# esologic/GANce

Hardware: AMD Instinct MI355X
Metric: synthesized frames/sec at 1024x1024 config-f (higher is better)
Workload: dtype f32 (bf16x3 split operands, 6 terms, fp32 accumulate)

## Files before the change

gance_amd/csrc/upfir_split.hip:

```cpp

#include <hip/hip_runtime.h>

#include <algorithm>
#include <cstdlib>
#include <cstring>
#include <type_traits>

#include "kernels.h"

#ifndef GANCE_UPFIRS_ABLATE
#define GANCE_UPFIRS_ABLATE 0
#endif

namespace gance {

namespace {

typedef float f32x4 __attribute__((ext_vector_type(4)));
typedef float f32x2 __attribute__((ext_vector_type(2)));
typedef unsigned u32x4 __attribute__((ext_vector_type(4)));
typedef unsigned u32x2 __attribute__((ext_vector_type(2)));
typedef __bf16 bf16x8 __attribute__((ext_vector_type(8)));
typedef __bf16 bf16x2 __attribute__((ext_vector_type(2)));
typedef __attribute__((address_space(3))) void* lds_ptr_t;

constexpr int kBM = 16;
constexpr int kKC = 32;
constexpr int kSW = 64;
constexpr int kTH = 8;
constexpr int kRows = kTH + 1;
constexpr int kPlanes = 12;
constexpr int kPlaneStride = 80;
constexpr int kSlotUnits = kPlanes * kPlaneStride;
constexpr int kRing = 3;
constexpr int kHaloCols = 4;
constexpr int kHaloUnits = kRows * kHaloCols * kPlanes;
constexpr int kHaloTasks = kRows * kHaloCols * 4;
#ifndef GANCE_UPFIRS_WEAVE
#define GANCE_UPFIRS_WEAVE 2
#endif
#ifndef GANCE_UPFIRS_MIN_SEG_ROWS
#define GANCE_UPFIRS_MIN_SEG_ROWS 16
#endif
#ifndef GANCE_UPFIRS_DEPTH
#define GANCE_UPFIRS_DEPTH 6
#endif
constexpr int kDepth = GANCE_UPFIRS_DEPTH;
constexpr int kCarryRows = 3;
constexpr int kPassCh = 4;
constexpr int kPassRows = 8;
constexpr float kSqrt2f = 1.4142135623730951f;
static_assert((2 * kRows) % kDepth == 0 && kDepth + 2 < kRows && kRows % kRing == 0, "ring slots and staging registers rotate with the unrolled rows of a chunk pair");

template <int NT>
struct Geo {
    static constexpr int kSW = 64 / NT;
    static constexpr int kBMB = kBM * NT;
    static constexpr int kTC = kSW / 16;
    static constexpr int kPW = 4 / NT;
    static constexpr int kTW = 2 * kSW + 4;
    static constexpr int kCG = kSW / 2;
    static constexpr int kRG = 64 / NT / kCG;
    static constexpr int kFR = kPassRows / kRG;
    static constexpr int kWin = kFR + 3;
    static constexpr int kCarryFloats = kBMB * kCarryRows * kTW;
    static constexpr int kStageFloats = kPassCh * NT * kPassRows * kTW;
    static constexpr int kNzPieces = 2 * kPassRows * 2 * kSW / 256;
    static constexpr int kWUnits = NT == 1 ? 27 * 64 : 0;
};

constexpr size_t kRingBytes = (size_t)kRing * kSlotUnits * 16;
constexpr size_t kHaloBytes = (size_t)2 * kHaloUnits * 16;
template <int NT>
constexpr size_t lds_bytes(int cin) {
    using G = Geo<NT>;
    return kRingBytes + kHaloBytes + (size_t)G::kWUnits * 16 +
           sizeof(float) * ((size_t)G::kStageFloats + G::kNzPieces * 256 + G::kCarryFloats + cin + 3 * G::kBMB);
}

__host__ __device__ constexpr int tap_cls(int t) { return t < 4 ? 0 : (t < 6 ? 1 : (t < 8 ? 2 : 3)); }
__host__ __device__ constexpr int tap_dy(int t) { return (t == 2 || t == 3 || t == 5) ? 1 : 0; }
__host__ __device__ constexpr int tap_dx(int t) { return (t == 1 || t == 3 || t == 7) ? 1 : 0; }

__device__ __forceinline__ void lds_barrier() {
    asm volatile("s_waitcnt lgkmcnt(0)" ::: "memory");
    __builtin_amdgcn_s_barrier();
    asm volatile("" ::: "memory");
}

__device__ __forceinline__ int fresh_lane() {
    int l;
    asm volatile("v_mbcnt_lo_u32_b32 %0, -1, 0\n\tv_mbcnt_hi_u32_b32 %0, -1, %0" : "=v"(l));
    return l;
}

__device__ __forceinline__ int ring_column(int P) {
    return ((P >> 2) & 3) | ((((P >> 4) ^ P) & 1) << 2) | (((P >> 1) & 1) << 3) | ((P & 1) << 4) | (P & 32);
}
constexpr int kEdgeColumn = 64;

__device__ __forceinline__ void split_pair(float a, float b, unsigned& p0, unsigned& p1, unsigned& p2) {
    auto pack = [](float lo, float hi) { return __builtin_bit_cast(unsigned, __builtin_convertvector(f32x2{lo, hi}, bf16x2)); };
    p0 = pack(a, b);
    const float ra = a - __builtin_bit_cast(float, p0 << 16), rb = b - __builtin_bit_cast(float, p0 & 0xffff0000u);
    p1 = pack(ra, rb);
    const float sa = ra - __builtin_bit_cast(float, p1 << 16), sb = rb - __builtin_bit_cast(float, p1 & 0xffff0000u);
    p2 = pack(sa, sb);
}

__device__ __forceinline__ void split_unit(const unsigned (&raw)[8], u32x4 (&part)[3]) {
    unsigned w[3][4];
    if (GANCE_UPFIRS_ABLATE & 1) {
#pragma unroll
        for (int q = 0; q < 3; ++q) part[q] = u32x4{raw[q], raw[q + 1], raw[q + 2], raw[q + 3]};
        return;
    }
#pragma unroll
    for (int e = 0; e < 4; ++e) split_pair(__builtin_bit_cast(float, raw[2 * e]), __builtin_bit_cast(float, raw[2 * e + 1]), w[0][e], w[1][e], w[2][e]);
#pragma unroll
    for (int q = 0; q < 3; ++q) part[q] = u32x4{w[q][0], w[q][1], w[q][2], w[q][3]};
}

}

template <int NT, bool kPre, bool kNoise>
__device__ __forceinline__ void upfirs_body(const UpFirArgs& p) {
    using G = Geo<NT>;
    constexpr int kSW = G::kSW, kBMB = G::kBMB, kTC = G::kTC, kPW = G::kPW, kTW = G::kTW, kCG = G::kCG, kRG = G::kRG, kFR = G::kFR,
                  kWin = G::kWin, kCarryFloats = G::kCarryFloats, kStageFloats = G::kStageFloats, kNzPieces = G::kNzPieces;
    extern __shared__ __attribute__((aligned(16))) unsigned char smem_raw[];
    u32x4* const ring = reinterpret_cast<u32x4*>(smem_raw);
    u32x4* const halo = ring + kRing * kSlotUnits;
    u32x4* const w_lds = halo + 2 * kHaloUnits;
    float* const stage = reinterpret_cast<float*>(w_lds + G::kWUnits);
    float* const nz_lds = stage + kStageFloats;
    float* const carry = nz_lds + kNzPieces * 256;
    float* const s_lds = carry + kCarryFloats;
    float* const d_lds = s_lds + (kPre ? 0 : p.Cin);
    float* const b_lds = d_lds + kBMB;
    float* const sn_lds = b_lds + kBMB;

    const int tid = threadIdx.x;
    const int wave = __builtin_amdgcn_readfirstlane(tid >> 6);
    const int lane = tid & 63;
    const int n16 = lane & 15, kg = lane >> 4;
    const int ct = NT == 1 ? 0 : wave / kTC, tc = NT == 1 ? wave : wave % kTC;

    int id;
    {
        const int v = blockIdx.x, nwg = p.total_blocks;
        const int q = nwg >> 3, r = nwg & 7, xcd = v & 7;
        id = (xcd < r ? xcd * (q + 1) : r * (q + 1) + (xcd - r) * q) + (v >> 3);
    }
    const int m_tile = id % p.m_tiles;
    id /= p.m_tiles;
    const int strip = id % p.strips;
    id /= p.strips;
    const int seg = id % p.segs;
    const int b = id / p.segs;
    const int m0 = m_tile * kBMB;
    const int X0 = strip * kSW;
    const int H = p.H, W = p.W;
    const int Hp = H + 2, Wp = W + 8;
    const int HpWp4 = Hp * Wp * 4;
    const int chunks = p.Cin / kKC;
    const int steps = H / kTH;
    const int s_begin = seg * (p.rows_per_seg / kTH), s_end = s_begin + p.rows_per_seg / kTH;
    const int s_first = seg > 0 ? s_begin - 1 : s_begin;

    const __amdgpu_buffer_rsrc_t x_rsrc =
        __builtin_amdgcn_make_buffer_rsrc((void*)(p.x + (size_t)b * p.x_b_stride), 0, p.Cin * Hp * Wp * 4, 0x00020000);
    const __amdgpu_buffer_rsrc_t w_rsrc = __builtin_amdgcn_make_buffer_rsrc(
        (void*)(reinterpret_cast<const unsigned char*>(p.w) + (size_t)(m_tile * NT + ct) * chunks * 27 * 1024), 0, chunks * 27 * 1024, 0x00020000);

    const int st_pair = lane >> 4, st_g = lane & 15;
    u32x4* const ring_w = ring + wave * kPlaneStride + ring_column(4 * st_g + st_pair);
    unsigned* const ring_wn = reinterpret_cast<unsigned*>(ring + wave * kPlaneStride + ring_column(NT == 2 ? 2 * st_g + (st_pair & 1) : st_g)) +
                              (NT == 2 ? 2 * (st_pair >> 1) : st_pair);
    const int m_pos = 16 * tc + n16;
    const u32x4* const ring_r0 = ring + kg * kPlaneStride + ring_column(m_pos);
    const u32x4* const ring_r1 = ring + kg * kPlaneStride + (m_pos > 0 ? ring_column(m_pos - 1) : kEdgeColumn);
    const bool edge_copy = wave == 3 && lane < kPlanes;
    const int e_unit = lane % kPlanes;
    u32x4* const ring_e = ring + (e_unit >> 2) * 4 * kPlaneStride + (e_unit & 3) * kPlaneStride + (edge_copy ? kEdgeColumn : 66 + wave);
    const u32x4* const halo_e = halo + e_unit;
    const u32x4* const halo_r = halo + ((n16 & 7) * kHaloCols + 2 * (n16 >> 3)) * kPlanes + kg;
    const u32x4* const halo_f = halo + ((kRows - 1) * kHaloCols + 2 * (n16 >> 3)) * kPlanes + kg;
    const int st_voff = (2 * st_pair * Hp * Wp + X0 + 4 + kPW * st_g) * 4;
    unsigned st[kDepth][8];
    auto stage_load = [&](unsigned(&dst)[8], int chunk, int brow, bool in_loop = false) {
        if ((GANCE_UPFIRS_ABLATE & 4) && in_loop) return;
        const int soff = ((chunk * kKC + wave * 8) * Hp + brow) * Wp * 4;
#pragma unroll
        for (int e = 0; e < 2; ++e) {
            if constexpr (kPW == 4) {
                const u32x4 q4 = __builtin_amdgcn_raw_buffer_load_b128(x_rsrc, st_voff, soff + e * HpWp4, 0);
#pragma unroll
                for (int c = 0; c < 4; ++c) dst[2 * c + e] = q4[c];
            } else if constexpr (kPW == 2) {
                const u32x2 q2 = __builtin_amdgcn_raw_buffer_load_b64(x_rsrc, st_voff, soff + e * HpWp4, 0);
                dst[e] = q2[0];
                dst[2 + e] = q2[1];
            } else {
                dst[e] = __builtin_amdgcn_raw_buffer_load_b32(x_rsrc, st_voff, soff + e * HpWp4, 0);
            }
        }
    };
    auto scale_pair = [&](unsigned(&raw)[8], int chunk) {
        if constexpr (!kPre) {
            const f32x2 s2 = *reinterpret_cast<const f32x2*>(s_lds + chunk * kKC + 8 * wave + 2 * st_pair);
#pragma unroll
            for (int c = 0; c < kPW; ++c) {
                raw[2 * c] = __builtin_bit_cast(unsigned, __builtin_bit_cast(float, raw[2 * c]) * s2[0]);
                raw[2 * c + 1] = __builtin_bit_cast(unsigned, __builtin_bit_cast(float, raw[2 * c + 1]) * s2[1]);
            }
        }
    };
    auto transpose_rows = [](u32x4& u) {
        auto a02 = __builtin_amdgcn_permlane32_swap(u[0], u[2], false, false);
        auto a13 = __builtin_amdgcn_permlane32_swap(u[1], u[3], false, false);
        auto b01 = __builtin_amdgcn_permlane16_swap(a02[0], a13[0], false, false);
        auto b23 = __builtin_amdgcn_permlane16_swap(a02[1], a13[1], false, false);
        u = u32x4{b01[0], b01[1], b23[0], b23[1]};
    };
    auto scale8 = [&](unsigned(&raw)[8], int chunk, int group) {
        if constexpr (!kPre) {
            const f32x4 s0 = *reinterpret_cast<const f32x4*>(s_lds + chunk * kKC + group * 8);
            const f32x4 s1 = *reinterpret_cast<const f32x4*>(s_lds + chunk * kKC + group * 8 + 4);
#pragma unroll
            for (int e = 0; e < 4; ++e) {
                raw[e] = __builtin_bit_cast(unsigned, __builtin_bit_cast(float, raw[e]) * s0[e]);
                raw[4 + e] = __builtin_bit_cast(unsigned, __builtin_bit_cast(float, raw[4 + e]) * s1[e]);
            }
        }
    };
    auto stage_store = [&](unsigned(&raw)[8], int slot, int chunk) {
        scale_pair(raw, chunk);
        if constexpr (NT == 1) {
            u32x4 part[3];
            split_unit(raw, part);
#pragma unroll
            for (int q = 0; q < 3; ++q) transpose_rows(part[q]);
#pragma unroll
            for (int q = 0; q < 3; ++q)
                if (!(GANCE_UPFIRS_ABLATE & 16)) ring_w[slot * kSlotUnits + q * 4 * kPlaneStride] = part[q];
        } else {
            unsigned w[3][kPW];
#pragma unroll
            for (int c = 0; c < kPW; ++c) split_pair(__builtin_bit_cast(float, raw[2 * c]), __builtin_bit_cast(float, raw[2 * c + 1]), w[0][c], w[1][c], w[2][c]);
#pragma unroll
            for (int q = 0; q < 3; ++q) {
                unsigned* const dst = ring_wn + 4 * (slot * kSlotUnits + q * 4 * kPlaneStride);
                if constexpr (NT == 2) {
                    const auto s = __builtin_amdgcn_permlane16_swap(w[q][0], w[q][1], false, false);
                    *reinterpret_cast<u32x2*>(dst) = u32x2{s[0], s[1]};
                } else {
                    *dst = w[q][0];
                }
            }
        }
    };
    auto edge_store = [&](int slot, int hbuf, int hrow) { if (!(GANCE_UPFIRS_ABLATE & 64)) ring_e[slot * kSlotUnits] = halo_e[hbuf * kHaloUnits + (hrow * kHaloCols + 1) * kPlanes]; };
    const int h_task = tid < kHaloTasks ? tid : tid - kHaloTasks;
    const int h_col = h_task & 3, h_kg = (h_task >> 2) & 3, h_row = h_task >> 4;
    const int h_voff = ((h_kg * 8 * Hp + h_row) * Wp + X0 + 2 + (h_col & 1) + (h_col >> 1) * (kSW + 1)) * 4;
    u32x4* const halo_w = halo + (h_row * kHaloCols + h_col) * kPlanes + h_kg;
    unsigned hraw[8];
    auto halo_load = [&](int step, int chunk) {
        const int soff = (chunk * kKC * Hp + kTH * step) * Wp * 4;
#pragma unroll
        for (int e = 0; e < 8; ++e) hraw[e] = __builtin_amdgcn_raw_buffer_load_b32(x_rsrc, h_voff, soff + e * HpWp4, 0);
    };
    auto halo_store = [&](int chunk, int buf) {
        scale8(hraw, chunk, h_kg);
        u32x4 part[3];
        split_unit(hraw, part);
#pragma unroll
        for (int q = 0; q < 3; ++q) halo_w[buf * kHaloUnits + q * 4] = part[q];
    };

    u32x4 A[9][3];
    const int a_voff = lane * 16;
    auto weights_dma = [&](int chunk) {
#pragma unroll
        for (int k = 0; k < 7; ++k)
            if (k < 6 || wave < 3)
                __builtin_amdgcn_raw_ptr_buffer_load_lds(w_rsrc, (lds_ptr_t)(w_lds + (wave + 4 * k) * 64), 16, lane * 16, (chunk * 27 + wave + 4 * k) * 1024, 0, 0);
    };
    const u32x4* const w_r = w_lds + lane;
    auto read_a3 = [&](int t, u32x4(&dst)[3]) {
#pragma unroll
        for (int q = 0; q < 3; ++q) dst[q] = w_r[(t * 3 + q) * 64];
    };
    auto load_a3 = [&](int chunk, int t, u32x4(&dst)[3]) {
#pragma unroll
        for (int q = 0; q < 3; ++q) dst[q] = __builtin_amdgcn_raw_buffer_load_b128(w_rsrc, a_voff, (chunk * 27 + t * 3 + q) * 1024, 0);
    };

    u32x4 Bf[2][2][3];
    auto load_b = [&](int slot, u32x4(&dst)[2][3]) {
#pragma unroll
        for (int q = 0; q < 3; ++q) {
            dst[0][q] = ring_r0[slot * kSlotUnits + q * 4 * kPlaneStride];
            dst[1][q] = ring_r1[slot * kSlotUnits + q * 4 * kPlaneStride];
        }
    };

    stage_load(st[0], 0, kTH * s_first + 0);
    stage_load(st[1], 0, kTH * s_first + 1);
    load_a3(0, 0, A[0]);
    halo_load(s_first, 0);
    if constexpr (!kPre)
        for (int i = tid; i < p.Cin; i += 256) s_lds[i] = p.s[(size_t)b * p.s_stride + i];
    if (tid < kBMB) {
        d_lds[tid] = p.d[(size_t)b * p.d_stride + m0 + tid];
        b_lds[tid] = p.bias[m0 + tid];
        sn_lds[tid] = p.s_next != nullptr ? p.s_next[(size_t)b * p.s_stride + m0 + tid] : 1.0f;
    }
    for (int i = tid; i < kCarryFloats; i += 256) carry[i] = 0.f;
    if constexpr (NT > 1)
        for (int i = tid; i < kPassCh * NT * kPassRows; i += 256) stage[i * kTW] = stage[i * kTW + 2 * kSW + 2] = stage[i * kTW + 2 * kSW + 3] = 0.f;
#pragma unroll
    for (int t = 1; t < 9; ++t) load_a3(0, t, A[t]);
    if constexpr (!kPre) lds_barrier();
    stage_store(st[0], 0, 0);
    stage_store(st[1], 1, 0);
    halo_store(0, 0);
#pragma unroll
    for (int r = 2; r < 2 + kDepth; ++r) stage_load(st[r % kDepth], 0, kTH * s_first + r);
    lds_barrier();
    edge_store(0, 0, 0);
    edge_store(1, 0, 1);
    lds_barrier();
    load_b(0, Bf[0]);

    const int OW = 2 * W, OWp = OW + 8;
    const long long oplane = (long long)(2 * H + 2) * OWp;
    const __amdgpu_buffer_rsrc_t o_rsrc = __builtin_amdgcn_make_buffer_rsrc(
        (void*)(p.out + ((size_t)b * p.Cout + m0) * oplane - 2 * OWp), 0, 0x7fffffff, 0x00020000);
    const __amdgpu_buffer_rsrc_t nz_rsrc = __builtin_amdgcn_make_buffer_rsrc(
        (void*)(kNoise ? p.noise + (size_t)b * p.noise_b_stride : nullptr), 0, kNoise ? (2 * H) * (2 * W) * 4 : 0, 0x00020000);
    const float ns2 = p.noise_strength * kSqrt2f;

    constexpr int kTerms[6][2] = {{2, 0}, {0, 2}, {1, 1}, {1, 0}, {0, 1}, {0, 0}};
    constexpr int kTapTurn[9] = {0, 4, 6, 8, 2, 5, 1, 7, 3};

#pragma unroll 1
    for (int si = s_first; si < s_end; ++si) {
        const int y0 = kTH * si;
        const bool last_step = si + 1 == steps;
        const bool priming = si < s_begin;
        f32x4 acc[kTH][4];
#pragma unroll
        for (int r = 0; r < kTH; ++r)
#pragma unroll
            for (int c = 0; c < 4; ++c) acc[r][c] = f32x4{0.f, 0.f, 0.f, 0.f};
        f32x4 accf[2] = {f32x4{0.f, 0.f, 0.f, 0.f}, f32x4{0.f, 0.f, 0.f, 0.f}};
        f32x4 acch[NT == 1 ? 1 : 2] = {}, acchf = f32x4{0.f, 0.f, 0.f, 0.f};

        auto run_chunk = [&](auto parity, const int chunk) {
            constexpr int ab = decltype(parity)::value;
            const int n_chunk = chunk + 1 < chunks ? chunk + 1 : 0;
            const int n_step = chunk + 1 < chunks ? si : (last_step ? si : si + 1);
#pragma unroll
            for (int j = 0; j < kRows; ++j) {
                const int cur = (j + ab) & 1;
                if (NT == 1 && j == 0) weights_dma(n_chunk);
                if (j == 0) halo_load(n_step, n_chunk);
                if (j == 4) halo_store(n_chunk, ab ^ 1);
                load_b((j + 1) % kRing, Bf[cur ^ 1]);
                edge_store((j + 2) % kRing, j + 2 < kRows ? ab : ab ^ 1, (j + 2) % kRows);
                stage_store(st[(kRows * ab + j + 2) % kDepth], (j + 2) % kRing, j + 2 < kRows ? chunk : n_chunk);
                stage_load(st[(kRows * ab + j + 2) % kDepth], j + 2 + kDepth < kRows ? chunk : n_chunk, kTH * (j + 2 + kDepth < kRows ? si : n_step) + (j + 2 + kDepth) % kRows, true);
                if (j + 1 < kRows) {
#pragma unroll
                    for (int term = 0; term < ((GANCE_UPFIRS_ABLATE & 8) ? 0 : 6); ++term)
#pragma unroll
                        for (int k = 0; k < 9; ++k) {
                            const int t = kTapTurn[k];
                            const int row = tap_dy(t) ? j : j - 1;
                            if (row < 0 || row >= kTH) continue;
                            acc[row][tap_cls(t)] = __builtin_amdgcn_mfma_f32_16x16x32_bf16(
                                __builtin_bit_cast(bf16x8, A[t][kTerms[term][1]]), __builtin_bit_cast(bf16x8, Bf[cur][tap_dx(t)][kTerms[term][0]]),
                                acc[row][tap_cls(t)], 0, 0, 0);
                        }
#pragma unroll
                    for (int i = 0; i < 54; ++i) {
                        if (i >= (j == 0 ? 18 : 54)) break;
                        __builtin_amdgcn_sched_group_barrier(0x008, 1, 0);
                        __builtin_amdgcn_sched_group_barrier(0x092, GANCE_UPFIRS_WEAVE, 0);
                    }
                } else {
                    constexpr int kOrder[9] = {2, 3, 5, 0, 1, 4, 6, 7, 8};
#pragma unroll
                    for (int i = 0; i < 9; ++i) {
                        const int t = kOrder[i];
                        if (!tap_dy(t)) {
#pragma unroll
                            for (int term = 0; term < 6; ++term)
                                acc[kTH - 1][tap_cls(t)] = __builtin_amdgcn_mfma_f32_16x16x32_bf16(
                                    __builtin_bit_cast(bf16x8, A[t][kTerms[term][1]]), __builtin_bit_cast(bf16x8, Bf[cur][tap_dx(t)][kTerms[term][0]]),
                                    acc[kTH - 1][tap_cls(t)], 0, 0, 0);
                        } else if (last_step) {
#pragma unroll
                            for (int term = 0; term < 6; ++term)
                                accf[tap_cls(t)] = __builtin_amdgcn_mfma_f32_16x16x32_bf16(
                                    __builtin_bit_cast(bf16x8, A[t][kTerms[term][1]]), __builtin_bit_cast(bf16x8, Bf[cur][tap_dx(t)][kTerms[term][0]]),
                                    accf[tap_cls(t)], 0, 0, 0);
                        }
                        const int hc = NT == 1 ? 0 : tap_cls(t) >> 1;
                        const bool halo_mine = NT == 1 ? wave == tap_cls(t) : (tap_dx(t) && (tap_cls(t) & 1) == 0 && (kTC == 1 || tc == hc));
                        if (halo_mine && !(GANCE_UPFIRS_ABLATE & 64)) {
                            u32x4 hf[3];
#pragma unroll
                            for (int q = 0; q < 3; ++q) hf[q] = halo_r[ab * kHaloUnits + ((1 - tap_dy(t)) * kHaloCols + 1 - tap_dx(t)) * kPlanes + q * 4];
#pragma unroll
                            for (int term = 0; term < 6; ++term)
                                acch[hc] = __builtin_amdgcn_mfma_f32_16x16x32_bf16(__builtin_bit_cast(bf16x8, A[t][kTerms[term][1]]),
                                                                                    __builtin_bit_cast(bf16x8, hf[kTerms[term][0]]), acch[hc], 0, 0, 0);
                            if (last_step && tap_dy(t)) {
#pragma unroll
                                for (int q = 0; q < 3; ++q) hf[q] = halo_f[ab * kHaloUnits + (1 - tap_dx(t)) * kPlanes + q * 4];
#pragma unroll
                                for (int term = 0; term < 6; ++term)
                                    acchf = __builtin_amdgcn_mfma_f32_16x16x32_bf16(__builtin_bit_cast(bf16x8, A[t][kTerms[term][1]]),
                                                                                    __builtin_bit_cast(bf16x8, hf[kTerms[term][0]]), acchf, 0, 0, 0);
                            }
                        }
                        if constexpr (NT == 1) read_a3(t, A[t]);
                        else load_a3(n_chunk, t, A[t]);
                    }
                }
                if (NT == 1 && j == kRows - 2) asm volatile("s_waitcnt vmcnt(24)" ::: "memory");
                if (!(GANCE_UPFIRS_ABLATE & 32)) lds_barrier();
            }
        };
#pragma unroll 1
        for (int chunk = 0; chunk < chunks; chunk += 2) {
            run_chunk(std::integral_constant<int, 0>{}, chunk);
            run_chunk(std::integral_constant<int, 1>{}, chunk + 1);
        }

        const int elane = fresh_lane();
        const int en16 = elane & 15, eq4 = elane >> 4;
        const int dump_base = (4 * ct + eq4) * (kPassRows * kTW) + 32 * tc + 2 * en16 + 1;
        const int hpy = wave >> 1, hpx = wave & 1;
        const int fsub = NT == 1 ? 0 : elane / (64 / NT), flane = NT == 1 ? elane : elane % (64 / NT);
        const int fc = NT == 1 ? wave : wave * NT + fsub;
        const int fch = NT == 1 ? fc : 16 * (fc >> 2) + (fc & 3);
        const int cg = flane % kCG;
        const int rg = flane / kCG;
        const int o_voff = (int)((fch * oplane + (long long)(kFR * rg) * OWp + 4 * cg) * 4);

        auto run_passes = [&](auto flush_tag) {
            constexpr bool kFlush = decltype(flush_tag)::value;
            const int ys = kFlush ? H : y0;
            if (kNoise) {
#pragma unroll
                for (int i = 0; i < (kNzPieces + 3) / 4; ++i) {
                    if (kNzPieces % 4 != 0 && wave + 4 * i >= kNzPieces) break;
                    const int f = (wave + 4 * i) * 256 + 4 * elane;
                    const int row = f / (2 * kSW), col = f % (2 * kSW);
                    __builtin_amdgcn_raw_ptr_buffer_load_lds(nz_rsrc, (lds_ptr_t)(nz_lds + (wave + 4 * i) * 256), 16,
                                                             ((2 * ys - 2 + row) * OW + 2 * X0 + col) * 4, 0, 0, 0);
                }
                asm volatile("s_waitcnt vmcnt(0)" ::: "memory");
            }
            constexpr int kRowPasses = kFlush ? 1 : 2;
#pragma unroll
            for (int rw = 0; rw < kRowPasses; ++rw) {
                const int oy0 = 2 * (ys + 4 * rw) - 2;
                const int r_lo = max(0, -oy0);
                const int r_hi = priming ? 0 : min(kPassRows, 2 * H - oy0);
#pragma unroll
                for (int g = 0; g < 4; ++g) {
                    if constexpr (kFlush) {
#pragma unroll
                        for (int c = 0; c < 4; ++c) stage[dump_base + (c >> 1) * kTW + (c & 1)] = c < 2 ? accf[c][g] : 0.f;
                        if constexpr (NT == 1) {
                            if (en16 == 0 || en16 == 8) {
                                const int side = en16 >> 3;
                                if (hpy == 0 && (side == 1 || hpx == 1)) stage[eq4 * (kPassRows * kTW) + (side ? 2 * kSW + 1 + hpx : 0)] = acchf[g];
                                if (hpy == 1 && (side == 1 || hpx == 1)) stage[eq4 * (kPassRows * kTW) + kTW + (side ? 2 * kSW + 1 + hpx : 0)] = 0.f;
                            }
                        } else if (en16 == 8 && tc == 0) {
                            stage[(4 * ct + eq4) * (kPassRows * kTW) + 2 * kSW + 1] = acchf[g];
                            stage[(4 * ct + eq4) * (kPassRows * kTW) + kTW + 2 * kSW + 1] = 0.f;
                        }
                    } else {
#pragma unroll
                        for (int r4 = 0; r4 < 4; ++r4)
#pragma unroll
                            for (int c = 0; c < 4; ++c) stage[dump_base + (2 * r4 + (c >> 1)) * kTW + (c & 1)] = acc[4 * rw + r4][c][g];
                        const int row = en16 & 7, side = en16 >> 3;
                        if constexpr (NT == 1) {
                            if ((side == 1 || hpx == 1) && row / 4 == rw)
                                stage[eq4 * (kPassRows * kTW) + (2 * (row % 4) + hpy) * kTW + (side ? 2 * kSW + 1 + hpx : 0)] = acch[0][g];
                        } else if (side == 1 && row / 4 == rw) {
#pragma unroll
                            for (int h = 0; h < 2; ++h)
                                if (kTC == 1 || tc == h) stage[(4 * ct + eq4) * (kPassRows * kTW) + (2 * (row % 4) + h) * kTW + 2 * kSW + 1] = acch[h][g];
                        }
                    }
                    lds_barrier();

                    const int ch = 4 * g + fch;
                    const float dsc = d_lds[ch] * kSqrt2f;
                    const float kh0 = 0.25f * dsc, kh1 = 0.75f * dsc;
                    const float bias2 = b_lds[ch] * kSqrt2f;
                    const float lr6 = 0.6f * sn_lds[ch], lr4 = 0.4f * sn_lds[ch];
                    const float* const win_lo = carry + ch * (kCarryRows * kTW) + (kFR * rg) * kTW + 4 * cg;
                    const float* const win_hi = stage + fc * (kPassRows * kTW) + (kFR * rg - kCarryRows) * kTW + 4 * cg;
                    f32x4 ta[kWin], tb[kWin];
#pragma unroll
                    for (int i = 0; i < kWin; ++i) {
                        const float* const rowp = (i < kCarryRows && kFR * rg + i < kCarryRows ? win_lo : win_hi) + i * kTW;
                        ta[i] = *reinterpret_cast<const f32x4*>(rowp);
                        tb[i] = *reinterpret_cast<const f32x4*>(rowp + 4);
                    }
                    {
                        const int o_soff = (int)((4 * g * oplane + (long long)(oy0 + 3) * OWp + 2 * X0 + 4) * 4);
#pragma unroll
                        for (int r = 0; r < kFR; ++r) {
                            const int rr = kFR * rg + r;
                            if (rr >= r_lo && rr < r_hi) {
                                f32x2 tv[4];
#pragma unroll
                                for (int c2 = 0; c2 < 4; ++c2) {
                                    auto pair = [&](int i) { return c2 < 2 ? f32x2{ta[i][2 * c2], ta[i][2 * c2 + 1]} : f32x2{tb[i][2 * c2 - 4], tb[i][2 * c2 - 3]}; };
                                    tv[c2] = 0.25f * pair(r) + 0.75f * pair(r + 1) + 0.75f * pair(r + 2) + 0.25f * pair(r + 3);
                                }
                                const float t[7] = {tv[0][0], tv[0][1], tv[1][0], tv[1][1], tv[2][0], tv[2][1], tv[3][0]};
                                f32x4 v;
#pragma unroll
                                for (int o = 0; o < 4; ++o) v[o] = fmaf(kh0, t[o + 3], fmaf(kh1, t[o + 2], fmaf(kh1, t[o + 1], fmaf(kh0, t[o], bias2))));
                                if (kNoise) v += ns2 * *reinterpret_cast<const f32x4*>(nz_lds + (kPassRows * rw + rr) * (2 * kSW) + 4 * cg);
#pragma unroll
                                for (int o = 0; o < 4; ++o) v[o] = fmaf(lr6, v[o], lr4 * __builtin_fabsf(v[o]));
                                if (!(GANCE_UPFIRS_ABLATE & 128)) __builtin_amdgcn_raw_buffer_store_b128(__builtin_bit_cast(u32x4, v), o_rsrc, o_voff, o_soff + r * OWp * 4, 0);
                                else asm volatile("" ::"v"(v));
                            }
                        }
                    }
                    lds_barrier();
                    if (!kFlush && rg == kRG - 1) {
                        float* const carry_w = carry + ch * (kCarryRows * kTW) + 4 * cg;
#pragma unroll
                        for (int i = 0; i < 3; ++i) {
                            *reinterpret_cast<f32x4*>(carry_w + i * kTW) = ta[kWin - 3 + i];
                            if (cg == kCG - 1) *reinterpret_cast<f32x4*>(carry_w + i * kTW + 4) = tb[kWin - 3 + i];
                        }
                    }
                }
            }
        };
        if (GANCE_UPFIRS_ABLATE & 2) {
            float sum = acch[0][0] + acchf[0] + accf[0][0] + accf[1][0];
#pragma unroll
            for (int r = 0; r < kTH; ++r)
#pragma unroll
                for (int c = 0; c < 4; ++c) sum += acc[r][c][0] + acc[r][c][3];
            if (sum == 12345.678f) p.out[tid] = sum;
            continue;
        }
        run_passes(std::false_type{});
        if (last_step) {
            lds_barrier();
            run_passes(std::true_type{});
        }
    }
}

bool upfirs_supported(int cin, int cout, int H, int W) {
    return H == W && W % kSW == 0 && H % kTH == 0 && cin % (2 * kKC) == 0 && cout % kBM == 0 && cin <= 512;
}

bool upfirs_narrow_supported(int cin, int cout, int H, int W) {
    return H == W && (W == 32 || W == 16) && H % kTH == 0 && cin % (2 * kKC) == 0 && cout % (kBM * (kSW / W)) == 0 && cin <= 512;
}

size_t upfirs_weight_floats(int cin, int cout) { return (size_t)(cout / kBM) * (cin / kKC) * 27 * 256; }

static unsigned short bf16_rne_host(float x) {
    unsigned u;
    std::memcpy(&u, &x, 4);
    u += 0x7fffu + ((u >> 16) & 1u);
    return (unsigned short)(u >> 16);
}
static float bf16_value_host(unsigned short h) {
    const unsigned u = (unsigned)h << 16;
    float f;
    std::memcpy(&f, &u, 4);
    return f;
}

void upfirs_arrange_weights(const float* w_in, int cin, int cout, const int* up_tap_weight, float* w_out) {
    unsigned short* const out = reinterpret_cast<unsigned short*>(w_out);
    const int m_tiles = cout / kBM, chunks = cin / kKC;
    for (int mt = 0; mt < m_tiles; ++mt)
        for (int ch = 0; ch < chunks; ++ch)
            for (int t = 0; t < 9; ++t)
                for (int k = 0; k < kKC; ++k)
                    for (int m = 0; m < kBM; ++m) {
                        const int channel = 4 * (m & 3) + (m >> 2);
                        const float v = w_in[((size_t)up_tap_weight[t] * cin + ch * kKC + k) * cout + mt * kBM + channel];
                        unsigned short part[3];
                        part[0] = bf16_rne_host(v);
                        const float r1 = v - bf16_value_host(part[0]);
                        part[1] = bf16_rne_host(r1);
                        part[2] = bf16_rne_host(r1 - bf16_value_host(part[1]));
                        for (int q = 0; q < 3; ++q)
                            out[((((((size_t)mt * chunks + ch) * 9 + t) * 3 + q) * 4 + k / 8) * 16 + m) * 8 + k % 8] = part[q];
                    }
}

void upfirs_plan(int B, int cout, int H, int W, int num_cus, UpFirArgs* a) {
    a->step_rows = kTH;
    a->stagger_phases = 1;
    a->stagger_ticks = 0;
    a->debug_flags = 0;
    if (W < kSW) {
        a->m_tiles = cout / (kBM * (kSW / W));
        a->strips = 1;
        a->segs = 1;
        a->rows_per_seg = H;
        a->total_blocks = B * a->m_tiles;
        return;
    }
    a->m_tiles = cout / kBM;
    a->strips = W / kSW;
    static const bool segments = [] { const char* v = std::getenv("GANCE_TUNE_UPFIR_SPLIT_SEGS"); return !(v && std::atoi(v) == 0); }();
    int segs = 1;
    const int base = B * a->m_tiles * a->strips;
    long long best = (long long)((base + num_cus - 1) / num_cus) * H;
    for (int n = 2; segments && H / n >= GANCE_UPFIRS_MIN_SEG_ROWS && (H / n) % kTH == 0 && base * (n / 2) < num_cus; n *= 2) {
        const long long cost = (long long)((base * n + num_cus - 1) / num_cus) * (H / n + kTH);
        if (cost < best) best = cost, segs = n;
    }
    a->segs = segs;
    a->rows_per_seg = H / segs;
    a->total_blocks = base * segs;
}

__global__ __launch_bounds__(256, 1) void upfirs_fused_kernel(const UpFirArgs p) { upfirs_body<1, false, false>(p); }
__global__ __launch_bounds__(256, 1) void upfirs_fused_noise_kernel(const UpFirArgs p) { upfirs_body<1, false, true>(p); }
__global__ __launch_bounds__(256, 1) void upfirs_fused_pre_kernel(const UpFirArgs p) { upfirs_body<1, true, false>(p); }
__global__ __launch_bounds__(256, 1) void upfirs_fused_pre_noise_kernel(const UpFirArgs p) { upfirs_body<1, true, true>(p); }
__global__ __launch_bounds__(256, 1) void upfirs_w32_fused_kernel(const UpFirArgs p) { upfirs_body<2, false, false>(p); }
__global__ __launch_bounds__(256, 1) void upfirs_w32_fused_noise_kernel(const UpFirArgs p) { upfirs_body<2, false, true>(p); }
__global__ __launch_bounds__(256, 1) void upfirs_w32_fused_pre_kernel(const UpFirArgs p) { upfirs_body<2, true, false>(p); }
__global__ __launch_bounds__(256, 1) void upfirs_w32_fused_pre_noise_kernel(const UpFirArgs p) { upfirs_body<2, true, true>(p); }
__global__ __launch_bounds__(256, 1) void upfirs_w16_fused_kernel(const UpFirArgs p) { upfirs_body<4, false, false>(p); }
__global__ __launch_bounds__(256, 1) void upfirs_w16_fused_noise_kernel(const UpFirArgs p) { upfirs_body<4, false, true>(p); }
__global__ __launch_bounds__(256, 1) void upfirs_w16_fused_pre_kernel(const UpFirArgs p) { upfirs_body<4, true, false>(p); }
__global__ __launch_bounds__(256, 1) void upfirs_w16_fused_pre_noise_kernel(const UpFirArgs p) { upfirs_body<4, true, true>(p); }

hipError_t launch_upfir_split(const UpFirArgs& args, hipStream_t stream) {
    using Kernel = void (*)(const UpFirArgs);
    static const Kernel kernels[3][4] = {
        {upfirs_fused_kernel, upfirs_fused_noise_kernel, upfirs_fused_pre_kernel, upfirs_fused_pre_noise_kernel},
        {upfirs_w32_fused_kernel, upfirs_w32_fused_noise_kernel, upfirs_w32_fused_pre_kernel, upfirs_w32_fused_pre_noise_kernel},
        {upfirs_w16_fused_kernel, upfirs_w16_fused_noise_kernel, upfirs_w16_fused_pre_kernel, upfirs_w16_fused_pre_noise_kernel}};
    static size_t (*const lds_of[3])(int) = {lds_bytes<1>, lds_bytes<2>, lds_bytes<4>};
    static PerDeviceInt ready;
    int unused = 0;
    const hipError_t e = ready.get(
        [&](int, int* value) {
            *value = 1;
            for (int gi = 0; gi < 3; ++gi)
                for (int i = 0; i < 4; ++i) {
                    const hipError_t err = hipFuncSetAttribute(reinterpret_cast<const void*>(kernels[gi][i]), hipFuncAttributeMaxDynamicSharedMemorySize,
                                                               (int)lds_of[gi](i >= 2 ? 0 : 512));
                    if (err != hipSuccess) return err;
                }
            return hipSuccess;
        },
        &unused);
    if (e != hipSuccess) return e;
    const int gi = args.W % kSW == 0 ? 0 : (args.W == 32 ? 1 : 2);
    const bool narrow = gi != 0;
    if (!(narrow ? upfirs_narrow_supported(args.Cin, args.Cout, args.H, args.W) : upfirs_supported(args.Cin, args.Cout, args.H, args.W)) || args.segs < 1 ||
        args.rows_per_seg * args.segs != args.H || args.rows_per_seg % kTH != 0 || args.total_blocks != args.B * args.m_tiles * args.strips * args.segs ||
        (narrow && (args.segs != 1 || args.strips != 1 || args.m_tiles * kBM * (kSW / args.W) != args.Cout)))
        return hipErrorInvalidValue;
    const int pre = args.input_prescaled ? 1 : 0, noise = args.noise != nullptr ? 1 : 0;
    hipLaunchKernelGGL(kernels[gi][2 * pre + noise], dim3(args.total_blocks), dim3(256), lds_of[gi](pre ? 0 : args.Cin), stream, args);
    return hipGetLastError();
}

}
```

Baseline: 1476.

## Defer last-chunk weight LDS reads past epilogue and add interior-pass specialization

For the single-tile path, the final chunk's row loop no longer rereads the next chunk's weights from LDS into registers. Those reads are issued after the epilogue passes, which shortens register live ranges during the epilogue and moves the LDS traffic out of the last MMA row. An optional interior-pass variant (off by default, EPI bit 2) drops the row-bounds checks. The acch staging store is made unconditional by redirecting unused lanes to a padding column, which removes a branch. The code is split into more template instantiations, which adds complexity and may change register allocation.

```diff
diff --git a/gance_amd/csrc/upfir_split.hip b/gance_amd/csrc/upfir_split.hip
--- a/gance_amd/csrc/upfir_split.hip
+++ b/gance_amd/csrc/upfir_split.hip
@@ -10,6 +10,9 @@
 
 #ifndef GANCE_UPFIRS_ABLATE
 #define GANCE_UPFIRS_ABLATE 0
+#endif
+#ifndef GANCE_UPFIRS_EPI
+#define GANCE_UPFIRS_EPI 1
 #endif
 
 namespace gance {
@@ -280,6 +283,7 @@
     };
 
     u32x4 A[9][3];
+    constexpr bool kLateWeights = NT == 1 && (GANCE_UPFIRS_EPI & 1);
     const int a_voff = lane * 16;
     auto weights_dma = [&](int chunk) {
 #pragma unroll
@@ -358,12 +362,13 @@
         f32x4 accf[2] = {f32x4{0.f, 0.f, 0.f, 0.f}, f32x4{0.f, 0.f, 0.f, 0.f}};
         f32x4 acch[NT == 1 ? 1 : 2] = {}, acchf = f32x4{0.f, 0.f, 0.f, 0.f};
 
-        auto run_chunk = [&](auto parity, const int chunk) {
-            constexpr int ab = decltype(parity)::value;
+        auto run_chunk = [&](auto parity, const int chunk, auto j0_tag, auto j1_tag, auto late_tag) {
+            constexpr int ab = decltype(parity)::value, kJ0 = decltype(j0_tag)::value, kJ1 = decltype(j1_tag)::value;
+            constexpr bool kLateA = decltype(late_tag)::value;
             const int n_chunk = chunk + 1 < chunks ? chunk + 1 : 0;
             const int n_step = chunk + 1 < chunks ? si : (last_step ? si : si + 1);
 #pragma unroll
-            for (int j = 0; j < kRows; ++j) {
+            for (int j = kJ0; j < kJ1; ++j) {
                 const int cur = (j + ab) & 1;
                 if (NT == 1 && j == 0) weights_dma(n_chunk);
                 if (j == 0) halo_load(n_step, n_chunk);
@@ -427,7 +432,7 @@
                                                                                     __builtin_bit_cast(bf16x8, hf[kTerms[term][0]]), acchf, 0, 0, 0);
                             }
                         }
-                        if constexpr (NT == 1) read_a3(t, A[t]);
+                        if constexpr (NT == 1) { if constexpr (!kLateA) read_a3(t, A[t]); }
                         else load_a3(n_chunk, t, A[t]);
                     }
                 }
@@ -437,8 +442,18 @@
         };
 #pragma unroll 1
         for (int chunk = 0; chunk < chunks; chunk += 2) {
-            run_chunk(std::integral_constant<int, 0>{}, chunk);
-            run_chunk(std::integral_constant<int, 1>{}, chunk + 1);
+            constexpr std::integral_constant<int, 0> c0{};
+            constexpr std::integral_constant<int, 1> c1{};
+            constexpr std::integral_constant<int, kRows - 1> c8{};
+            constexpr std::integral_constant<int, kRows> c9{};
+            run_chunk(c0, chunk, c0, c9, std::false_type{});
+            if constexpr (kLateWeights) {
+                run_chunk(c1, chunk + 1, c0, c8, std::false_type{});
+                if (chunk + 2 < chunks) run_chunk(c1, chunk + 1, c8, c9, std::false_type{});
+                else run_chunk(c1, chunk + 1, c8, c9, std::true_type{});
+            } else {
+                run_chunk(c1, chunk + 1, c0, c9, std::false_type{});
+            }
         }
 
         const int elane = fresh_lane();
@@ -452,8 +467,10 @@
         const int rg = flane / kCG;
         const int o_voff = (int)((fch * oplane + (long long)(kFR * rg) * OWp + 4 * cg) * 4);
 
-        auto run_passes = [&](auto flush_tag) {
-            constexpr bool kFlush = decltype(flush_tag)::value;
+        auto run_passes = [&](auto flush_tag, auto interior_tag) {
+            constexpr bool kFlush = decltype(flush_tag)::value, kInterior = decltype(interior_tag)::value;
+            static_assert(!(kFlush && kInterior), "the flush pass is an edge case");
+            if constexpr (kInterior) asm volatile("; upfirs interior passes begin" ::: "memory");
             const int ys = kFlush ? H : y0;
             if (kNoise) {
 #pragma unroll
@@ -470,10 +487,11 @@
 #pragma unroll
             for (int rw = 0; rw < kRowPasses; ++rw) {
                 const int oy0 = 2 * (ys + 4 * rw) - 2;
-                const int r_lo = max(0, -oy0);
-                const int r_hi = priming ? 0 : min(kPassRows, 2 * H - oy0);
+                const int r_lo = kInterior ? 0 : max(0, -oy0);
+                const int r_hi = kInterior ? kPassRows : (priming ? 0 : min(kPassRows, 2 * H - oy0));
 #pragma unroll
                 for (int g = 0; g < 4; ++g) {
+                    if constexpr (kInterior) asm volatile("; upfirs interior pass" ::: "memory");
                     if constexpr (kFlush) {
 #pragma unroll
                         for (int c = 0; c < 4; ++c) stage[dump_base + (c >> 1) * kTW + (c & 1)] = c < 2 ? accf[c][g] : 0.f;
@@ -494,8 +512,8 @@
                             for (int c = 0; c < 4; ++c) stage[dump_base + (2 * r4 + (c >> 1)) * kTW + (c & 1)] = acc[4 * rw + r4][c][g];
                         const int row = en16 & 7, side = en16 >> 3;
                         if constexpr (NT == 1) {
-                            if ((side == 1 || hpx == 1) && row / 4 == rw)
-                                stage[eq4 * (kPassRows * kTW) + (2 * (row % 4) + hpy) * kTW + (side ? 2 * kSW + 1 + hpx : 0)] = acch[0][g];
+                            const bool mine = (side == 1 || hpx == 1) && row / 4 == rw;
+                            stage[eq4 * (kPassRows * kTW) + (2 * (row % 4) + hpy) * kTW + (mine ? (side ? 2 * kSW + 1 + hpx : 0) : kTW - 1)] = acch[0][g];
                         } else if (side == 1 && row / 4 == rw) {
 #pragma unroll
                             for (int h = 0; h < 2; ++h)
@@ -523,7 +541,7 @@
 #pragma unroll
                         for (int r = 0; r < kFR; ++r) {
                             const int rr = kFR * rg + r;
-                            if (rr >= r_lo && rr < r_hi) {
+                            if (kInterior || (rr >= r_lo && rr < r_hi)) {
                                 f32x2 tv[4];
 #pragma unroll
                                 for (int c2 = 0; c2 < 4; ++c2) {
@@ -553,6 +571,14 @@
                     }
                 }
             }
+            if constexpr (kInterior) asm volatile("; upfirs interior passes end" ::: "memory");
+        };
+        auto read_late_weights = [&] {
+            if constexpr (kLateWeights) {
+#pragma unroll
+                for (int t = 0; t < 9; ++t) read_a3(t, A[t]);
+                lds_barrier();
+            }
         };
         if (GANCE_UPFIRS_ABLATE & 2) {
             float sum = acch[0][0] + acchf[0] + accf[0][0] + accf[1][0];
@@ -561,13 +587,16 @@
 #pragma unroll
                 for (int c = 0; c < 4; ++c) sum += acc[r][c][0] + acc[r][c][3];
             if (sum == 12345.678f) p.out[tid] = sum;
+            read_late_weights();
             continue;
         }
-        run_passes(std::false_type{});
+        if ((GANCE_UPFIRS_EPI & 2) && !priming && si > 0) run_passes(std::false_type{}, std::true_type{});
+        else run_passes(std::false_type{}, std::false_type{});
         if (last_step) {
             lds_barrier();
-            run_passes(std::true_type{});
+            run_passes(std::true_type{}, std::false_type{});
         }
+        read_late_weights();
     }
 }
 
```

Measured after the change: 1487, median of 6. About the same (+0.8%).
